# TLeconte/vdlm2dec

Measured on AMD Instinct MI355X. Metric: IQ MS/s demodulated (8 ch, 2 MS/s cs16) + CRC-pass frame parity vs ref, higher is better.
Workload: dtype f32

## Files before the change

vdlm2dec_amd/csrc/vdl2gpu.hip:

```cpp
#include "vdl2gpu_kernels.h"
#include "vdl2gpu_blocks.h"

#include <algorithm>
#include <cerrno>
#include <cmath>
#include <cstdio>
#include <cstdlib>
#include <chrono>
#include <cstring>
#include <mutex>
#include <new>
#include <string>
#include <type_traits>
#include <vector>

extern "C" void sincosf(float, float *, float *);

#define HIPCHK(h, expr)                                                                         \
	do {                                                                                    \
		hipError_t e__ = (expr);                                                        \
		if (e__ != hipSuccess) {                                                        \
			(h)->err = std::string(#expr) + ": " + hipGetErrorString(e__);          \
			return VDL2GPU_EHIP;                                                    \
		}                                                                               \
// ... 174 lines not shown
	uint64_t last_redo_push = 0;
	unsigned long long *d_dbg = nullptr;
	HeadTap *d_headtap = nullptr;
	unsigned *d_headtap_n = nullptr;
	unsigned headtap_cap = 0;
	uint64_t total_in = 0;
	uint64_t test_epoch = 0;
	unsigned test_ticket0 = 0;
	uint64_t pushes = 0;
	uint64_t overflowed = 0;
	std::vector<PushTiming> pending;
	std::vector<PushTiming> free_ev;
	vdl2gpu_timing_t tm{};
	RecQueue ready;
	std::vector<uint64_t> ready_idx;
	Slab slab[VDL2_NSLAB];
	unsigned slab_cap = 0;
	size_t ready_pos = 0;
	bool frames_on = false;
	unsigned *d_k4tab = nullptr;
	unsigned *d_fcnt = nullptr;
	unsigned frame_cap = 0;

	std::vector<uint8_t> fready;
	std::vector<size_t> fready_idx;
	size_t fready_pos = 0;
	uint64_t frames_dropped = 0;
	vdl2gpu_burst_t *h_pin = nullptr;
	bool col_on[VDL2_NCOL] = {};
	double lev_k = 1.0;
	unsigned *h_pin_cnt = nullptr;
	unsigned *d_pin_cnt = nullptr;
	unsigned pin_recs = 0;
	bool failed = false;
	std::string err;
	double hprof[8] = {0, 0, 0, 0, 0, 0, 0, 0};
	bool hprof_on = false;
	uint64_t hprof_push0 = 0;
	struct {
		bool no_k1_fast = false;
		bool no_tail = false;
		bool no_whole_pp = false;
		double table_fill = 0.90;
		bool k1_pp = false;
		bool debug_counters = false;
		bool split_fixed = false;
		int k1f_nfam = 0;
		int verify2_wg = 8;
		int k1_nsub = 0;
#ifdef VDL2GPU_TESTHOOKS
		int test_item_grid = 0;
		int test_item_common = 0;
		int test_item_verify = 0;
		int test_reg_cap = 0, test_seg_cap = 0, test_vis_cap = 0, test_win_cap = 0, test_merge_cap = 0, test_slog_cap = 0, test_stage_dyn = 0;
#endif
	} knob;
	struct Back {
		bool valid = false;
		K2Params k2{};
		int64_t J = 0;
		int par = 0, ring = 0, slab = 0;
		bool serial = false, two_streams = false;
		bool spec = false;
		unsigned tiles = 0;
		size_t pt_index = 0;
	} back;
	hipStream_t fstream = nullptr;
	LaterEvent k1_ev;
	hipEvent_t f_tail = nullptr;
	bool last_two_streams = false;
	int64_t last_J = 0;
	double st_scan = 0, st_cluster = 0, st_resolve = 0, st_demod = 0, st_other = 0, st_k1 = 0;
	uint64_t st_pushes = 0;
};

int LaterEvent::record(vdl2gpu_t *h, hipStream_t s) { HIPCHK(h, hipEventRecord(ev, s)); recorded = true; return VDL2GPU_OK; }
int LaterEvent::wait(vdl2gpu_t *h, hipStream_t s) const { if (recorded) HIPCHK(h, hipStreamWaitEvent(s, ev, 0)); return VDL2GPU_OK; }
int LaterEvent::sync(vdl2gpu_t *h) const { if (recorded) HIPCHK(h, hipEventSynchronize(ev)); return VDL2GPU_OK; }

extern "C" unsigned int reversebits(const unsigned int bits, const int n)
{
	unsigned int r = 0;
	for (int i = 0; i < n; ++i)
		r |= ((bits >> i) & 1u) << (n - 1 - i);
	return r;
}

extern "C" int vdl2gpu_lo_len(unsigned sdrinrate)
{
	unsigned a = sdrinrate, b = 25000u;
	while (b) {
		const unsigned t = a % b;
		a = b;
		b = t;
	}
	return a ? (int)(sdrinrate / a) : 0;
}

extern "C" int vdl2gpu_lo_table(unsigned sdrinrate, int fo_hz, float *out_re_im, int max_complex)
{
	const int L = vdl2gpu_lo_len(sdrinrate);
	if (L <= 0 || L > max_complex)
		return VDL2GPU_EINVAL;
	const float w = (float)((double)((float)fo_hz / (float)sdrinrate) * 2.0 * M_PI);
	for (int n = 0; n < L; ++n) {
		const float y = (float)(-n) * w;
		float sn, cs;
// ... 358 lines not shown
	ALLOC_TABLE(h, sel_list2, SC * VDL2_SEL_CAP * sizeof(unsigned));
	ALLOC_TABLE(h, regs, SC * VDL2_REG_CAP * sizeof(int2));
	ALLOC_TABLE(h, segs, SC * VDL2_SEG_CAP * sizeof(Seg));
	ALLOC_TABLE(h, fail, SC * sizeof(int));
	ALLOC_TABLE(h, redo, SC * sizeof(int));
	ALLOC_TABLE(h, cs_out, SC * sizeof(ChanState));
	ALLOC_TABLE(h, skey, SC * VDL2_CAND_CAP * sizeof(int));
	ALLOC_TABLE(h, sidx, SC * VDL2_CAND_CAP * sizeof(unsigned short));
	ALLOC_TABLE(h, prim, SC * VDL2_CAND_CAP * sizeof(unsigned short));
	ALLOC_TABLE(h, seeds, SC * VDL2_CAND_CAP * sizeof(int));
	for (TableSet &t : h->set) {
		DEV_ALLOC(h, t.k2.onchain, SC * VDL2_CAND_CAP);
		DEV_ALLOC(h, t.k2.slog, SC * VDL2_SLOG_CAP * sizeof(K2Slog));
		DEV_ALLOC(h, t.k2.win, SC * VDL2_WIN_CAP * sizeof(int2));
	}
	ALLOC_TABLE(h, items, SC * h->item_cap * sizeof(K2aItem));
	return VDL2GPU_OK;
}

static void fill_set_params(vdl2gpu_t *h)
{
	for (int r = 0; r < VDL2_NSET; ++r) {
		K2Params &k = h->set[r].k2;
		k.dec = h->d_dec[r];
		k.cap = h->cap;
		k.nbch = h->C;
		k.nstreams = h->S;
		k.ss = h->d_ss;
		k.cs = h->d_cs;
		k.cfg = h->d_cfg;
		k.pn = h->d_pn;
		k.pn8 = h->d_pn8;
		k.sel_mode = 0;
		k.stage_cap = h->stage_cap;
		k.outc_total_redo = h->d_outc + 8;
		k.rec_cap = h->rec_cap;
		k.probe_r = 0;
		k.prim_drop = h->prim_drop;
		k.dbg = h->knob.debug_counters ? h->d_dbg : nullptr;
		k.headtap = h->d_headtap;
		k.headtap_n = h->d_headtap_n;
		k.headtap_cap = h->headtap_cap;
		k.full_scan = h->full_scan;
#ifdef VDL2GPU_TESTHOOKS
		k.test_noregion = (h->cfg.flags & VDL2GPU_F_TEST_NOREGION) ? 1 : 0;
		{
			auto lim = [](int hook, int size) { return hook > 0 && hook < size ? hook : size; };
			k.lim_reg = lim(h->knob.test_reg_cap, VDL2_REG_CAP);
			k.lim_seg = lim(h->knob.test_seg_cap, VDL2_SEG_CAP);
			k.lim_vis = lim(h->knob.test_vis_cap, K2C_VIS);
			k.lim_win = lim(h->knob.test_win_cap, VDL2_WIN_CAP);
			k.lim_merge = lim(h->knob.test_merge_cap, K2S_MERGE);
			k.lim_slog = lim(h->knob.test_slog_cap, VDL2_SLOG_CAP);
			k.stage_cap = h->stage_cap - STAGE_DYN_SLOTS + (unsigned)lim(h->knob.test_stage_dyn, (int)STAGE_DYN_SLOTS);
		}
#endif
		k.round = 0;
		k.item_cap = h->item_cap;
		k.item_priv = h->item_priv;
		k.drain_slot = -1;
	}
}

static const int PART_SECONDS = 36, TEST_PART_NUM = 4, TEST_PART_DEN = 3;

static int create_impl(vdl2gpu_t *h)
{
	const vdl2gpu_config_t &cfg = h->cfg;
	int ndev = 0;
	if (hipGetDeviceCount(&ndev) != hipSuccess || ndev <= 0 || cfg.device >= ndev) {
		h->err = "no HIP device";
		return VDL2GPU_ENODEV;
	}
	HIPCHK(h, hipSetDevice(cfg.device));
	{
		hipDeviceProp_t prop;
		if (hipGetDeviceProperties(&prop, cfg.device) == hipSuccess && prop.multiProcessorCount > 0)
			h->n_cu = prop.multiProcessorCount;
		int occ = 0;
		if (hipOccupancyMaxActiveBlocksPerMultiprocessor(&occ, k2a_probe, K2A_THREADS, 0) == hipSuccess && occ > 0)
			h->probe_occ = occ;
	}
	int prio_lo = 0, prio_hi = 0;
	HIPCHK(h, hipDeviceGetStreamPriorityRange(&prio_lo, &prio_hi));
	NEW_STREAM(h, h->stream, &prio_hi);
	const int S = h->S, L = h->L;
	auto env_int = [](const char *name, int dflt) { const char *v = getenv(name); return v ? atoi(v) : dflt; };
	h->full_scan = ((cfg.flags & VDL2GPU_F_FULLSCAN) || getenv("VDL2GPU_FULL_SCAN")) ? 1 : 0;
	h->stage_every = std::max(1, env_int("VDL2GPU_STAGE_EVERY", h->stage_every));
	h->stage_dump = env_int("VDL2GPU_STAGE_DUMP", 0) != 0;
	if (h->stage_dump)
		h->stage_every = 1;
	h->k2d_grid = std::max(1, env_int("VDL2GPU_K2D_GRID", h->k2d_grid));
	h->knob.no_k1_fast = getenv("VDL2GPU_NO_K1_FAST") != nullptr;
	h->hprof_on = getenv("VDL2GPU_HOST_PROF") != nullptr;
	h->knob.no_tail = getenv("VDL2GPU_NO_TAIL") != nullptr;
	h->knob.no_whole_pp = getenv("VDL2GPU_NO_WHOLE_PP") != nullptr;
	h->knob.table_fill = std::min(100, std::max(10, env_int("VDL2GPU_TABLE_FILL", 90))) / 100.0;
	h->knob.k1_pp = getenv("VDL2GPU_K1_PP") != nullptr;
	h->knob.debug_counters = getenv("VDL2GPU_DEBUG_COUNTERS") != nullptr;
	h->knob.k1f_nfam = env_int("VDL2GPU_K1F_NFAM", 0);
	h->knob.verify2_wg = std::max(1, env_int("VDL2GPU_VERIFY2_WG", 8));
	h->knob.k1_nsub = env_int("VDL2GPU_K1_NSUB", 0);
#ifdef VDL2GPU_TESTHOOKS
	h->prim_drop = env_int("VDL2GPU_PRIM_DROP", 0);
	h->knob.test_item_grid = env_int("VDL2GPU_TEST_ITEM_GRID", 0);
	h->knob.test_item_common = env_int("VDL2GPU_TEST_ITEM_COMMON", 0);
	h->knob.test_item_verify = env_int("VDL2GPU_TEST_ITEM_VERIFY", 0);
	h->knob.test_reg_cap = env_int("VDL2GPU_TEST_REG_CAP", 0);
	h->knob.test_seg_cap = env_int("VDL2GPU_TEST_SEG_CAP", 0);
	h->knob.test_vis_cap = env_int("VDL2GPU_TEST_VIS_CAP", 0);
	h->knob.test_win_cap = env_int("VDL2GPU_TEST_WIN_CAP", 0);
	h->knob.test_merge_cap = env_int("VDL2GPU_TEST_MERGE_CAP", 0);
	h->knob.test_slog_cap = env_int("VDL2GPU_TEST_SLOG_CAP", 0);
	h->knob.test_stage_dyn = env_int("VDL2GPU_TEST_STAGE_DYN", 0);
#endif
	h->split_unit = ((cfg.flags & VDL2GPU_F_RTL_QUIRK) || h->sdrclk != 500 || h->L != 80) ? 32768 : K1F_PER_IN;
	if (!(cfg.flags & VDL2GPU_F_RTL_QUIRK) && h->split_unit == 32768 && (4 * h->sdrclk) % h->L == 0 && ((size_t)4 * h->sdrclk * h->sample_bytes) % 16 == 0)
		h->split_unit = (size_t)4 * h->sdrclk * ((32768 + (size_t)4 * h->sdrclk - 1) / ((size_t)4 * h->sdrclk));
	h->split_default = (size_t)((double)PART_SECONDS * (double)h->cfg.sdrinrate) / h->split_unit * h->split_unit;
	{
		const double max_frames = ((double)VDL2_MAXWG * K2A_VRUN - 4.0) * 2.0 * K2A_TS - 2.0 * K2A_TS - (double)VDL2_CARRY_FRAMES;
		const size_t max_part = (size_t)(max_frames * (double)h->sdrclk / 21.0) / h->split_unit * h->split_unit;
		h->split_default = std::min(h->split_default, max_part);
	}
	h->split_samples = std::max(h->split_unit, (size_t)(8.4 * (double)h->cfg.sdrinrate) / h->split_unit * h->split_unit);
#ifdef VDL2GPU_TESTHOOKS
	if (getenv("VDL2GPU_SPLIT_SAMPLES")) {
		h->split_samples = std::min((size_t)atoll(getenv("VDL2GPU_SPLIT_SAMPLES")), h->split_default * TEST_PART_NUM / TEST_PART_DEN);
		h->knob.split_fixed = true;
	}
#endif
	h->rounds_floor = 1;
	h->repair_rounds = env_int("VDL2GPU_REPAIR_ROUNDS", h->rounds_floor);
	h->force_serial = (cfg.flags & VDL2GPU_F_SERIAL) ? 1 : 0;
	h->quirk = (cfg.flags & VDL2GPU_F_RTL_QUIRK) ? 1 : 0;
	{
		const long long jmax = (long long)((21ull * cfg.max_push) / (unsigned)h->sdrclk) + 2;
		const long long jcap = (long long)PART_SECONDS * 84000 * TEST_PART_NUM / TEST_PART_DEN;
		const long long tiles_max = (VDL2_CARRY_FRAMES + std::min(jmax, jcap)) / K2A_TS + 2;
		const unsigned priv = (unsigned)std::min<long long>(VDL2_ITEM_PRIV, std::max<long long>(32768, (64 * tiles_max + 4095) / 4096 * 4096));
		h->item_priv = priv;
		h->item_cap = priv + std::max(priv / 2, 32768u);
	}
	h->k1_tbase.assign((size_t)S * 8, h->test_ticket0);
	h->cap = plane_frames(cfg.max_push, (unsigned)h->sdrclk);
	const size_t dec_bytes = (size_t)S * (size_t)h->cap * VDL2_CS * sizeof(float2);
	for (int r = 0; r < VDL2_NSET; ++r) {
		DEV_ALLOC(h, h->d_dec[r], dec_bytes);
		HIPCHK(h, hipMemsetAsync(h->d_dec[r], 0, dec_bytes, h->stream));
	}
	DEV_ALLOC(h, h->d_lo, (size_t)S * VDL2_CS * L * sizeof(float2));
	DEV_ALLOC(h, h->d_lo_ext, (size_t)S * VDL2_CS * (L + 48) * sizeof(float2));
	DEV_ALLOC(h, h->d_k1_tickets, (size_t)S * 21 * 8 * sizeof(unsigned));
	HIPCHK(h, hipMemsetAsync(h->d_k1_tickets, 0, (size_t)S * 21 * 8 * sizeof(unsigned), h->stream));
#ifdef VDL2GPU_TESTHOOKS
	if (h->test_ticket0) {
		const std::vector<unsigned> tk0((size_t)S * 21 * 8, h->test_ticket0);
		HIPCHK(h, hipMemcpyAsync(h->d_k1_tickets, tk0.data(), tk0.size() * sizeof(unsigned), hipMemcpyHostToDevice, h->stream));
		HIPCHK(h, hipStreamSynchronize(h->stream));
	}
#endif
	DEV_ALLOC(h, h->d_ss, (size_t)S * sizeof(StreamState));
	DEV_ALLOC(h, h->d_cs, (size_t)S * VDL2_CS * sizeof(ChanState));
	DEV_ALLOC(h, h->d_cfg, (size_t)S * VDL2_CS * sizeof(ChanCfg));
	DEV_ALLOC(h, h->d_pn, VDL2_PN_BITS);
	for (OutRing &rg : h->ring)
		DEV_ALLOC(h, rg.d_recs, (size_t)h->rec_cap * sizeof(vdl2gpu_burst_t));
// ... 994 lines not shown
	return VDL2GPU_OK;
}

static int enqueue_front(vdl2gpu_t *h, hipStream_t fs, long long dec_base, PushTiming &pt)
{
	vdl2gpu::Back &p = h->back;
	const int GS = h->S, par = p.par, ring = p.ring;
	const int64_t J = p.J;
	const bool serial = p.serial, two_streams = p.two_streams;
	TableSet &set = h->set[par];
	{
		KInitParams ki{};
		ki.ctl = set.k2.ctl + CTL_STAGE;
		ki.ctl_words = (int)(h->ctl_words - CTL_STAGE);
		ki.outc = h->d_outc + 2 * ring;
		ki.fail = set.k2.fail;
		ki.redo = set.k2.redo;
		ki.nsc = h->S * VDL2_CS;
		ki.fmask = set.k2.fmask;
		ki.fcnt = h->frames_on ? h->d_fcnt + 4 * ring : nullptr;
		hipLaunchKernelGGL(k_push_init, dim3(1), dim3(1024), 0, fs, ki);
	}
	TRY(mark(h, pt, E_SCAN_BEGIN, fs));
	K2Params k2 = set.k2;
	k2.J = J;
	k2.recs = h->ring[ring].d_recs;
	k2.levels = h->ring[ring].col<vdl2gpu_level_t>(COL_LEVEL);
	k2.soft = h->ring[ring].col<vdl2gpu_soft_t>(COL_SOFT);
	k2.carrier = h->ring[ring].col<vdl2gpu_carrier_t>(COL_CARRIER);
	k2.outc = h->d_outc + 2 * ring;
	k2.dec_base = dec_base;
	k2.scan_lo = dec_base + VDL2_HIST;
	k2.probe_par = (int)((dec_base + VDL2_HIST) & 1);
	k2.force_serial = serial ? 1 : 0;
	k2.sel_reserved = p.spec ? 1 : 0;
	if (h->d_headtap) {
		HIPCHK(h, hipStreamSynchronize(h->stream));
		HIPCHK(h, hipStreamSynchronize(h->pay_stream));
		HIPCHK(h, hipStreamSynchronize(h->copy_stream));
		HIPCHK(h, hipMemsetAsync(h->d_headtap_n, 0, sizeof(unsigned), fs));
	}
	const unsigned tiles = (unsigned)((VDL2_CARRY_FRAMES + J) / K2A_TS + 2);
	if (!serial) {
		ScanDrain pdrain, rdrain;
		{
			const unsigned want = h->full_scan ? tiles : tiles / 2 + 1;
			unsigned per = (unsigned)((h->n_cu * h->probe_occ + h->C * GS - 1) / (h->C * GS));
			per = per < 1 ? 1 : (per > want ? want : per);
			per = std::min<unsigned>(per, VDL2_MAXWG);
			TRY(launch_scan(h, SCAN_PROBE, k2, dim3(per, (unsigned)h->C, (unsigned)GS), fs, VDL2_SURV_PROBE,
					h->full_scan ? SURV_CANDS : SURV_PROBE, 0, (h->full_scan ? 4 : 1) * ((want + per - 1) / per), pdrain));
		}
		launch_per_channel(h, k2r_regions, K2R_NT, fs, k2, pdrain);
		TRY(launch_scan(h, SCAN_REGION, k2, dim3(128, (unsigned)h->C, (unsigned)GS), fs, VDL2_SURV_REGION, SURV_CANDS, 1, 2, rdrain));
		HIPCHK(h, hipGetLastError());
		launch_per_channel(h, k2s_sort, K2S_NT, fs, k2, rdrain);
	}
	TRY(mark(h, pt, E_FRONT_END, fs));
	HIPCHK(h, hipGetLastError());
	if (two_streams)
		HIPCHK(h, hipEventRecord(set.f_done, fs));
	{
		if (two_streams)
			TRY(h->set[set_after(par)].k2_done.wait(h, fs));
		K3Params k3{};
		k3.src = h->d_dec[par];
		k3.dst = h->d_dec[set_after(par)];
		k3.cap = h->cap;
		k3.nbch = h->C;
		k3.J = J;
		hipLaunchKernelGGL(k3_carry, dim3(24, (unsigned)h->C, (unsigned)GS), dim3(K3_THREADS), 0, fs, k3);
		HIPCHK(h, hipGetLastError());
		if (two_streams)
			HIPCHK(h, hipEventRecord(h->f_tail, fs));
		else
			TRY(h->k1_ev.record(h, fs));
	}
	p.valid = true;
	p.k2 = k2;
	p.tiles = tiles;
	p.pt_index = h->pending.size();
	return VDL2GPU_OK;
}

static int push_impl(vdl2gpu_t *h, const void *iq, size_t nsamples, size_t stream_stride_bytes, int memkind, bool wait_copy)
{
	if (!h || (!iq && nsamples))
		return VDL2GPU_EINVAL;
	if (nsamples == 0)
		return VDL2GPU_OK;
	if (nsamples > h->cfg.max_push)
		return VDL2GPU_EINVAL;
	if (h->S > 1 && stream_stride_bytes < nsamples * h->sample_bytes)
		return VDL2GPU_EINVAL;
	if (h->quirk && nsamples % 32768) {
		h->err = "VDL2GPU_F_RTL_QUIRK: every push must be whole 32768-sample blocks";
		return VDL2GPU_EINVAL;
	}
	HIPCHK(h, hipSetDevice(h->cfg.device));
	if (h->pending.size() >= 256) {
		HIPCHK(h, hipStreamSynchronize(h->fstream));
		HIPCHK(h, hipStreamSynchronize(h->stream));
		HIPCHK(h, hipStreamSynchronize(h->pay_stream));
		int rc = harvest_timing(h);
		if (rc)
			return rc;
	}
// ... 983 lines not shown
```

vdlm2dec_amd/csrc/vdl2gpu_scan.h:

```cpp
#ifndef VDL2GPU_SCAN_H
#define VDL2GPU_SCAN_H

#ifndef K2A_THREADS
#define K2A_THREADS 256
#endif
#ifndef K2A_TS
#define K2A_TS 1024
#endif
#ifndef K2A_WPE
#define K2A_WPE 6
#endif
#define K2A_POFF 132
#define K2A_XOFF (K2A_POFF + 16)
#define K2A_XMAX (2 * K2A_TS + K2A_XOFF)
#define K2X_WL 40
#define K2X_NT 256
#define K2X_CV 64
#define VDL2_ITEM_CAP 196608
#define VDL2_ITEM_PRIV 131072
#define VDL2_MAXWG 512
#define VDL2_REG_CAP 4096
#ifndef VDL2_REG_PAD
#define VDL2_REG_PAD 40
#endif
// ... 460 lines not shown
		v2f xe[10], xo[10];
#pragma unroll
		for (int i = 0; i < 5; ++i) {
			xe[2 * i] = e[i].xy;
			xe[2 * i + 1] = e[i].zw;
			xo[2 * i] = o[i].xy;
			xo[2 * i + 1] = o[i].zw;
		}
#pragma unroll
		for (int m = 0; m < 9; ++m) {
			acc0 = __builtin_elementwise_fma(xe[m], (v2f){mf[2 * m], mf[2 * m]}, acc0);
			acc1 = __builtin_elementwise_fma(xe[m + 1], (v2f){mf[2 * m], mf[2 * m]}, acc1);
			if (m < 8) {
				acc0 = __builtin_elementwise_fma(xo[m], (v2f){mf[2 * m + 1], mf[2 * m + 1]}, acc0);
				acc1 = __builtin_elementwise_fma(xo[m + 1], (v2f){mf[2 * m + 1], mf[2 * m + 1]}, acc1);
			}
		}
	} else {
		const v4f *pe = reinterpret_cast<const v4f *>(&sh.xs[q0]);
		v4f e[9];
#pragma unroll
		for (int i = 0; i < 9; ++i)
			e[i] = pe[i];
		v2f x[18];
#pragma unroll
		for (int i = 0; i < 9; ++i) {
			x[2 * i] = e[i].xy;
			x[2 * i + 1] = e[i].zw;
		}
#pragma unroll
		for (int j = 0; j < 17; ++j) {
			acc0 = __builtin_elementwise_fma(x[j], (v2f){mf[j], mf[j]}, acc0);
			acc1 = __builtin_elementwise_fma(x[j + 1], (v2f){mf[j], mf[j]}, acc1);
		}
	}
}

__device__ __forceinline__ v2f k2a_unit(v2f a)
{
	const float n2 = __fmaf_rn(a.x, a.x, a.y * a.y);
	v2f w = a * __frsqrt_rn(n2);
	if (!(n2 >= 1e-30f && n2 <= 1e30f)) {
		const float bad = (a.x == 0.0f && a.y == 0.0f) ? 0.0f : __builtin_nanf("");
		w = (v2f){1.0f + bad, bad};
	}
	return w;
}

__device__ __forceinline__ float k2a_lane_from(int byte_addr, float v)
{
	return __int_as_float(__builtin_amdgcn_ds_bpermute(byte_addr, __float_as_int(v)));
}

template <int S> __device__ void k2a_tile(K2aShared &sh, const K2Params &p, int sc, long long dec_base, long long nbase,
					   int cnt, unsigned rmask, int mode, long long chk_lo, long long chk_hi, int *fail,
					   int skip_r = -1, int skip_par = 0)
{
	const int tid = threadIdx.x;
	constexpr int PH = K2A_POFF / S;
	constexpr int LSTR = 8 / S;
	constexpr int E2 = 2 / S, E4 = 4 / S;
	constexpr int KH = LSTR / 2;
	constexpr int PPW = 64 - KH;
	constexpr int PPI = (K2A_THREADS / 64) * PPW;
	constexpr int NIT = ((K2A_TS + PH + 1) / 2 + PPI - 1) / PPI;
	constexpr int NL = (S * (K2A_TS - 1) + 1 + K2A_XOFF + K2A_THREADS - 1) / K2A_THREADS;
	static_assert(K2A_POFF == S * PH, "phase history must be a whole number of instants");
	float2 *const wu = (S != 1) ? sh.xs : sh.xs + K2A_WU1;
	const int nx = S * (cnt - 1) + 1 + K2A_XOFF;
	const bool prof = p.dbg && (mode == 2 || (mode == 0 && S == 1 && !p.full_scan && !p.full_round)) && tid == 0 && (blockIdx.x & 7) == 0;
	long long tq = prof ? clock64() : 0;
#define K2A_STAMP(slot) do { if (prof) { const long long tn = clock64(); sh.prof[slot] += (unsigned long long)(tn - tq); tq = tn; } } while (0)
	const int pbase = (S == 2) ? (tid & 1) * K2A_XODD + (tid >> 1) : tid;
	constexpr int pstep = K2A_THREADS / S;
	{
		const float2 *x = p.dec + (size_t)sc * p.cap + (nbase - K2A_XOFF - dec_base);
		float2 v[NL];
#pragma unroll
		for (int k = 0; k < NL; ++k)
			if (tid + k * K2A_THREADS < nx)
				v[k] = x[tid + k * K2A_THREADS];
		K2A_STAMP(12);
#pragma unroll
		for (int k = 0; k < NL; ++k)
			if (tid + k * K2A_THREADS < nx)
				sh.xs[pbase + k * pstep] = v[k];
	}
	K2A_STAMP(13);
	__syncthreads();
	K2A_STAMP(0);
	const int npairs = (cnt + PH + 1) / 2;
	const int wv = tid >> 6, ln = tid & 63;
	const int src_lane = (ln - KH) * 4;
#pragma unroll 1
	for (int r = 0; r < 4; ++r) {
		if (!(rmask & (1u << r)))
			continue;
		float mf[17];
#pragma unroll
		for (int j = 0; j < 17; ++j)
			mf[j] = __int_as_float(__builtin_amdgcn_readfirstlane(__float_as_int(sh.smf[r + 4 * j])));
		float4 hold[NIT];
#pragma unroll
		for (int it = 0; it < NIT; ++it) {
			const int pw = it * PPI + wv * PPW;
			if (pw >= npairs) {
				hold[it] = make_float4(0.0f, 0.0f, 0.0f, 0.0f);
				continue;
			}
			int q0 = 2 * (pw + ln - KH);
			q0 = q0 < 0 ? 0 : (q0 > K2A_TS + PH - 2 ? K2A_TS + PH - 2 : q0);
			v2f acc[2];
			k2a_fir2<S>(sh, q0, mf, acc[0], acc[1]);
			const v2f w0 = k2a_unit(acc[0]), w1 = k2a_unit(acc[1]);
			const float p0x = k2a_lane_from(src_lane, w0.x), p0y = k2a_lane_from(src_lane, w0.y);
			const float p1x = k2a_lane_from(src_lane, w1.x), p1y = k2a_lane_from(src_lane, w1.y);
			hold[it] = make_float4(__fmaf_rn(w0.x, p0x, w0.y * p0y), __fmaf_rn(w0.y, p0x, -(w0.x * p0y)),
					       __fmaf_rn(w1.x, p1x, w1.y * p1y), __fmaf_rn(w1.y, p1x, -(w1.x * p1y)));
			__builtin_amdgcn_sched_barrier(0);
		}
		K2A_STAMP(1);
		if (S != 1)
			__syncthreads();
		K2A_STAMP(2);
#pragma unroll
		for (int it = 0; it < NIT; ++it) {
			const int q0 = 2 * (it * PPI + wv * PPW + ln - KH);
			if (ln >= KH && q0 >= LSTR && q0 < cnt + PH)
				*reinterpret_cast<float4 *>(&wu[q0]) = hold[it];
		}
		K2A_STAMP(3);
		__syncthreads();
		unsigned npend = 0;
		for (int i0 = 0; i0 < cnt; i0 += K2A_THREADS) {
			const int i = i0 + tid;
			const int j = (i < cnt ? i : cnt - 1) + E2;
			const float2 *uq = &wu[PH - E4 + j - 15 * LSTR];
			float2 uu[16];
#pragma unroll
			for (int l = 0; l < 16; ++l)
				uu[l] = uq[l * LSTR];
			constexpr int kq[16] = {7, 4, 5, 3, 7, 6, 1, 3, 6, 0, 5, 2, 1, 2, 0, 4};
			v2f s4[4] = {{0.0f, 0.0f}, {0.0f, 0.0f}, {0.0f, 0.0f}, {0.0f, 0.0f}};
#pragma unroll
			for (int l = 0; l < 16; ++l) {
				const v2f u = {uu[l].x, uu[l].y};
				const int g = ((kq[l] & 1) << 1) | ((kq[l] >> 1) & 1);
				if (kq[l] & 4)
					s4[g] -= u;
				else
					s4[g] += u;
			}
			const v2f pa = {s4[0].x - s4[1].y, s4[0].y + s4[1].x};
			const v2f qa = {s4[2].x - s4[3].y, s4[2].y + s4[3].x};
			constexpr float RH = 0.70710678118654752f;
			const v2f acc = {__fmaf_rn(qa.x - qa.y, RH, pa.x), __fmaf_rn(qa.x + qa.y, RH, pa.y)};
			const float r2 = __fmaf_rn(acc.x, acc.x, acc.y * acc.y);
			bool pass = i < cnt && !(r2 <= VDL2_SCREEN_R2);
			if (mode == 0 && r == skip_r && (int)((nbase + S * (j - E4)) & 1) == skip_par)
				pass = false;
			const unsigned long long m = __ballot(pass);
			if (m != 0) {
				if (pass)
					sh.pend[wv][npend + __builtin_amdgcn_mbcnt_hi((unsigned)(m >> 32), __builtin_amdgcn_mbcnt_lo((unsigned)m, 0u))] =
						(unsigned short)(i | (!(r2 == r2) ? 0x8000 : 0));
				npend += (unsigned)__popcll(m);
			}
		}
		for (unsigned b = 0; b < npend; b += 64) {
			const bool on = b + (unsigned)ln < npend;
			const int e = on ? (int)sh.pend[wv][b + (unsigned)ln] : 0;
			const int j = (e & 0x3ff) + E2;
			const float2 *uq = &wu[PH - E4 + j - 15 * LSTR];
			float2 uu[16];
#pragma unroll
			for (int l = 0; l < 16; ++l)
				uu[l] = uq[l * LSTR];
			const long long n_abs = nbase + S * (j - E4);
			k2a_append(sh, p, sc, on, (int)(n_abs - dec_base), r, (mode == 1) ? (int)(chk_lo - dec_base) : 0,
				   (mode == 1) ? (int)(chk_hi - dec_base) : 0, uu, (e & 0x8000) != 0, mode, fail);
		}
		K2A_STAMP(4);
		K2A_STAMP(8);
		__syncthreads();
		K2A_STAMP(9);
		if (prof)
			sh.prof[11] += 1ull;
	}
#undef K2A_STAMP
}

__global__ __launch_bounds__(K2A_THREADS) __attribute__((amdgpu_waves_per_eu(K2A_WPE, 8)))
void k2a_probe(K2Params p)
{
	__shared__ K2aShared sh;
	const int c = blockIdx.y, s = (int)blockIdx.z;
	const int sc = s * VDL2_CS + c;
	const long long dec_base = p.dec_base;
	const long long avail_end = dec_base + VDL2_CARRY_FRAMES + p.J;
	if (p.force_serial)
		return;
	if (p.round > 0 && (!p.full_round || p.fail[sc] >= VDL2_VERIFIED))
		return;
	if (threadIdx.x < 16)
		sh.prof[threadIdx.x] = 0;
	k2a_tables(sh);
	if (p.full_scan || p.full_round) {
		const long long step = (long long)gridDim.x * K2A_TS;
		for (long long n0 = p.scan_lo + (long long)blockIdx.x * K2A_TS; n0 < avail_end; n0 += step) {
			const int nt = (int)((avail_end - n0 < K2A_TS) ? (avail_end - n0) : K2A_TS);
			k2a_tile<1>(sh, p, sc, dec_base, n0, nt, 0xfu, 0, 0, 0, nullptr);
		}
		k2a_tail(sh, sc);
		return;
	}
	const unsigned rmask = 1u << p.probe_r;
	const long long step = 2LL * gridDim.x * K2A_TS;
	for (long long n0 = p.scan_lo + 2LL * blockIdx.x * K2A_TS; n0 < avail_end; n0 += step) {
		const long long left = (avail_end - n0 + 1) / 2;
		const int nt = (int)(left < K2A_TS ? left : K2A_TS);
		k2a_tile<2>(sh, p, sc, dec_base, n0, nt, rmask, 2, 0, 0, nullptr);
	}
	k2a_tail(sh, sc);
	if (p.dbg && threadIdx.x < 16 && sh.prof[threadIdx.x])
		atomicAdd(p.dbg + 32 + threadIdx.x, sh.prof[threadIdx.x]);
}

#define WGS_NBK 2048
#define WGS_MAXB 48
struct WgSortShared {
	unsigned long long tmp[VDL2_CAND_CAP];
	unsigned start[WGS_NBK + 1], cur[WGS_NBK];
	unsigned part[64];
	unsigned maxb;
};

template <int NT> __device__ void wg_sort_u64(unsigned long long *keys, WgSortShared &ws, int n, int tshift, unsigned range)
{
	const int tid = threadIdx.x;
	int bsh = 0;
	while ((range >> bsh) >= WGS_NBK)
// ... 122 lines not shown
	for (int i = tid; i < ncand; i += K2R_NT)
		key64[i] = ((unsigned long long)(unsigned)seeds[i] << 16) | (unsigned)i;
	__syncthreads();
	wg_sort_u64<K2R_NT>(key64, ws, ncand, 16, (unsigned)(VDL2_CARRY_FRAMES + p.J));
	for (int i = tid; i < ncand; i += K2R_NT)
		key[i] = (int)(key64[i] >> 16);
	__syncthreads();
	{
		__shared__ int s_nreg;
		const int lo_lim = (int)(p.scan_lo - p.dec_base);
		const int hi_lim = (int)(VDL2_CARRY_FRAMES + p.J);
		int2 *regs = p.regs + (size_t)sc * VDL2_REG_CAP;
		if (tid == 0)
			s_nreg = 0;
		__syncthreads();
		for (int i = tid; i < ncand; i += K2R_NT) {
			if (i > 0 && key[i] - key[i - 1] <= VDL2_REG_GAP)
				continue;
			int j = i;
			while (j + 1 < ncand && key[j + 1] - key[j] <= VDL2_REG_GAP)
				++j;
			int lo = key[i] - VDL2_REG_PAD, hi = key[j] + VDL2_REG_PAD + 1;
			lo = lo < lo_lim ? lo_lim : lo;
			hi = hi > hi_lim ? hi_lim : hi;
			if (hi <= lo)
				continue;
			const int nchunk = (hi - lo + K2A_TS - 1) / K2A_TS;
			const int base = atomicAdd(&s_nreg, nchunk);
			for (int k = 0; k < nchunk; ++k)
				if (base + k < VDL2_REG_CAP) {
					const int q = lo + k * K2A_TS;
					regs[base + k] = make_int2(q, (hi - q < K2A_TS) ? hi - q : K2A_TS);
				}
		}
		__syncthreads();
#ifdef VDL2GPU_TESTHOOKS
		if (K2_REG_LIM(p) < VDL2_REG_CAP && s_nreg > K2_REG_LIM(p)) {
			const int n = s_nreg < VDL2_REG_CAP ? s_nreg : VDL2_REG_CAP, lim = K2_REG_LIM(p);
			for (int i = tid; i < n; i += K2R_NT)
				key64[i] = ((unsigned long long)(unsigned)regs[i].x << 32) | (unsigned)regs[i].y;
			__syncthreads();
			for (int i = tid; i < n; i += K2R_NT) {
				const int x = (int)(key64[i] >> 32);
				int rank = 0;
				for (int j = 0; j < n; ++j)
					rank += ((int)(key64[j] >> 32) < x) ? 1 : 0;
				const int k = (int)(((long long)rank * lim + n - 1) / n);
				if (k < lim && (int)((long long)k * n / lim) == rank)
					regs[k] = make_int2(x, (int)(key64[i] & 0xffffffffu));
			}
			__syncthreads();
		}
#endif
		if (tid == 0) {
			const int n = s_nreg;
			p.ctl[CTL_NREG0 + sc] = (unsigned)(n > K2_REG_LIM(p) ? K2_REG_LIM(p) : n);
			if (n > K2_REG_LIM(p))
				K2_COUNT(p, K2_DBG_ESC_REG);
			p.ctl[CTL_NSEED0 + sc] = 0;
		}
	}
}

#ifndef K2A_WPE_REGION
#define K2A_WPE_REGION 5
#endif
__global__ __launch_bounds__(K2A_THREADS) __attribute__((amdgpu_waves_per_eu(K2A_WPE_REGION, 8)))
void k2a_region(K2Params p)
{
	__shared__ K2aShared sh;
	const int c = blockIdx.y, s = (int)blockIdx.z;
	const int sc = s * VDL2_CS + c;
	if (p.force_serial || p.full_scan)
		return;
#ifdef VDL2GPU_TESTHOOKS
	if (p.test_noregion && p.round == 0)
		return;
#endif
	const unsigned nreg = p.ctl[CTL_NREG0 + sc];
	if (blockIdx.x >= nreg)
		return;
	const long long dec_base = p.dec_base;
	const int2 *regs = p.regs + (size_t)sc * VDL2_REG_CAP;
	const int skip_r = p.probe_r, skip_par = p.probe_par;
	if (threadIdx.x < 16)
		sh.prof[threadIdx.x] = 0;
	k2a_tables(sh);
	const bool prof = p.dbg && threadIdx.x == 0 && (blockIdx.x & 7) == 0;
	const long long t0 = prof ? clock64() : 0;
	for (unsigned k = blockIdx.x; k < nreg; k += gridDim.x) {
		const int2 rg = regs[k];
		k2a_tile<1>(sh, p, sc, dec_base, dec_base + rg.x, rg.y, 0xfu, 0, 0, 0, nullptr, skip_r, skip_par);
		if (prof)
			sh.prof[15] += (unsigned long long)rg.y;
	}
	const long long t1 = prof ? clock64() : 0;
	if (prof)
		sh.prof[12] += (unsigned long long)(t1 - t0);
	k2a_tail(sh, sc);
	if (p.dbg && threadIdx.x < 16 && sh.prof[threadIdx.x])
		atomicAdd(p.dbg + 48 + threadIdx.x, sh.prof[threadIdx.x]);
}

#ifndef K2A_VRUN
#define K2A_VRUN 4
#endif
#ifndef K2A_VGRID_RESIDENT
#define K2A_VGRID_RESIDENT 1
#endif
#define K2A_VITEMS 64

__device__ __forceinline__ int k2a_vseg(const Seg *segs, int k, int nseg, int p_lo, int t_end, int &lo, int &hi, int &r)
{
	lo = hi = r = 0;
	if (k >= nseg)
		return 0;
	const Seg g = segs[k];
	lo = g.lo > p_lo ? g.lo : p_lo;
	lo += (lo ^ g.lo) & 1;
	hi = g.hi < t_end ? g.hi : t_end;
	r = g.r & 3;
	if (g.hi <= g.lo || hi <= lo) {
		hi = lo;
		return 0;
	}
	return ((hi - lo + 1) / 2 + K2A_TS - 1) / K2A_TS;
}

__device__ __forceinline__ int k2a_vscan(int v, int *s_w, int &total)
{
	int incl = v;
	incl += __builtin_amdgcn_update_dpp(0, incl, 0x111, 0xf, 0xf, false);
	incl += __builtin_amdgcn_update_dpp(0, incl, 0x112, 0xf, 0xf, false);
	incl += __builtin_amdgcn_update_dpp(0, incl, 0x114, 0xf, 0xf, false);
	incl += __builtin_amdgcn_update_dpp(0, incl, 0x118, 0xf, 0xf, false);
	incl += __builtin_amdgcn_update_dpp(0, incl, 0x142, 0xa, 0xf, false);
	incl += __builtin_amdgcn_update_dpp(0, incl, 0x143, 0xc, 0xf, false);
	__syncthreads();
	if ((threadIdx.x & 63) == 63)
		s_w[threadIdx.x >> 6] = incl;
	__syncthreads();
	int base = 0, tot = 0;
#pragma unroll
	for (int w = 0; w < K2A_THREADS / 64; ++w) {
		const int t = s_w[w];
		base += (w < (int)(threadIdx.x >> 6)) ? t : 0;
		tot += t;
	}
	total = tot;
	return base + incl - v;
}

// ... 96 lines not shown
```

vdlm2dec_amd/csrc/vdl2gpu_types.h:

```cpp
#ifndef VDL2GPU_TYPES_H
#define VDL2GPU_TYPES_H


#include <hip/hip_runtime.h>
#include <stdint.h>
#include "vdl2_math.h"
#include "../../include/vdl2gpu.h"

#define VDL2_CS 8
#ifndef VDL2_NSET
#define VDL2_NSET 3
#endif
#define VDL2_NRING VDL2_NSET
#define VDL2_NSLAB (VDL2_NSET + 1)
static_assert(VDL2_NSET >= 3 && VDL2_NSET <= 4, "d_outc[] has the per-ring counters in front of the running totals at [8]; three bits of a record handle name its slab");
#define VDL2_HIST 160
#define VDL2_NPH 68
#define VDL2_STEADY 68
#define VDL2_MAXSYM 5456
#define VDL2_SERIAL_BELOW 4096
#define VDL2_CARRY_FRAMES 49152
#define VDL2_LONGEST_BURST 43592
#define VDL2_LEV_GUARD 512
#define VDL2_LEV_NEVAL 256
// ... 159 lines not shown
	Cluster *clusters;
	int2 *clhead;
	unsigned *ctl;
	BurstDesc *stage;
	unsigned *sel_list;
	unsigned *sel_list2;
	int sel_mode;
	unsigned stage_cap;
	vdl2gpu_burst_t *recs;
	vdl2gpu_level_t *levels;
	vdl2gpu_soft_t *soft;
	unsigned *outc;
	unsigned *outc_total_redo;
	unsigned *fmask;
	int full_round;
	int mini_round;
	int sel_reserved;
	unsigned rec_cap;
	int force_serial;
	int prim_drop;
	int full_scan;
	int test_noregion;
	int2 *regs;
	Seg *segs;
	int *fail;
	int *redo;
	int round;
	ChanState *cs_out;
	int *skey;
	unsigned short *sidx;
	unsigned short *prim;
	uint8_t *onchain;
	K2Slog *slog;
	int2 *win;
	int *seeds;
	struct K2aItem *items;
	unsigned item_cap;
	unsigned item_priv;
	int surv_pch, surv_nwg;
	int surv_common_cap;
	int surv_slot;
	int surv_mode;
	int surv_skip;
	int drain_slot;
	int drain_mode, drain_skip;
	int drain_pch, drain_nwg;
	unsigned long long *dbg;
	HeadTap *headtap;
	unsigned *headtap_n;
	unsigned headtap_cap;
	vdl2gpu_carrier_t *carrier;
#ifdef VDL2GPU_TESTHOOKS
	int lim_reg, lim_seg, lim_vis, lim_win, lim_merge, lim_slog;
#endif
};
#ifdef VDL2GPU_TESTHOOKS
#define K2_REG_LIM(p) ((p).lim_reg)
#define K2_SEG_LIM(p) ((p).lim_seg)
#define K2_VIS_LIM(p) ((p).lim_vis)
#define K2_WIN_LIM(p) ((p).lim_win)
#define K2_MERGE_LIM(p) ((p).lim_merge)
#define K2_SLOG_LIM(p) ((p).lim_slog)
enum { K2_DBG_ESC_REG = 64, K2_DBG_ESC_SEG, K2_DBG_ESC_VIS, K2_DBG_ESC_WIN, K2_DBG_ESC_MERGE, K2_DBG_ESC_SLOG, K2_DBG_ESC_STAGE,
       K2_DBG_INV_B_CLUSTER, K2_DBG_INV_B_DECODE, K2_DBG_INV_B_RECORD, K2_DBG_INV_A, K2_DBG_ESC_MERGE_SORT,
       K2_DBG_ESC_PATCH_ABANDON, K2_DBG_CHK_B_CLUSTER, K2_DBG_CHK_B_DECODE, K2_DBG_CHK_B_RECORD, K2_DBG_CHK_A };
#define VDL2_DBG_WORDS 96
#define K2_COUNT(p, slot) do { if ((p).dbg) atomicAdd((p).dbg + (slot), 1ull); } while (0)
#else
#define K2_REG_LIM(p) VDL2_REG_CAP
#define K2_SEG_LIM(p) VDL2_SEG_CAP
#define K2_VIS_LIM(p) K2C_VIS
#define K2_WIN_LIM(p) VDL2_WIN_CAP
#define K2_MERGE_LIM(p) K2S_MERGE
#define K2_SLOG_LIM(p) VDL2_SLOG_CAP
#define VDL2_DBG_WORDS 64
#define K2_COUNT(p, slot) do { } while (0)
#endif
#define CTL_OUT 0
#define CTL_OUT_OVF 1
#define CTL_STAGE 2
#define CTL_TICKET 3
#define CTL_STAGE_OVF 4
#define CTL_CAND0 8
#define CTL_NREG0 (CTL_CAND0 + 2 * p.nstreams * VDL2_CS)
#define CTL_NSEG0 (CTL_CAND0 + 3 * p.nstreams * VDL2_CS)
#define CTL_NSEL0 (CTL_CAND0 + 4 * p.nstreams * VDL2_CS)
#define CTL_NPRIM0 (CTL_CAND0 + 5 * p.nstreams * VDL2_CS)
#define CTL_NSEED0 (CTL_CAND0 + 6 * p.nstreams * VDL2_CS)
#define CTL_NCLUST0 (CTL_CAND0 + 7 * p.nstreams * VDL2_CS)
#define CTL_NSURV0 (CTL_CAND0 + 8 * p.nstreams * VDL2_CS)
enum { VDL2_SURV_PROBE = 0, VDL2_SURV_REGION = 1, VDL2_SURV_VERIFY = 2 , VDL2_SURV_FULL = 7, VDL2_SURV_SLOTS = 8 };
#define CTL_SELBASE0 (CTL_CAND0 + (8 + VDL2_SURV_SLOTS) * p.nstreams * VDL2_CS)
#define CTL_NSEL1 (CTL_CAND0 + (9 + VDL2_SURV_SLOTS) * p.nstreams * VDL2_CS)
#define CTL_SELBASE1 (CTL_CAND0 + (10 + VDL2_SURV_SLOTS) * p.nstreams * VDL2_CS)
#define CTL_NSURVLIM0 (CTL_CAND0 + (11 + VDL2_SURV_SLOTS) * p.nstreams * VDL2_CS)
#define CTL_NWIN0 (CTL_CAND0 + (11 + 2 * VDL2_SURV_SLOTS) * p.nstreams * VDL2_CS)
#define CTL_NSLOG0 (CTL_CAND0 + (12 + 2 * VDL2_SURV_SLOTS) * p.nstreams * VDL2_CS)
#define VDL2_CTL_WORDS(nsc) (CTL_CAND0 + (13 + 2 * VDL2_SURV_SLOTS) * (size_t)(nsc))
#define VDL2_WIN_CAP 32
#define VDL2_WIN_ALL 0xffffffffu
#define VDL2_SLOG_CAP 16

struct K3Params {
	const float2 *src;
	float2 *dst;
	long long cap;
	int nbch;
	long long J;
	StreamState *ss;
	const ChanState *cs;
	const unsigned *outc;
	const unsigned *fmask;
	const unsigned *fcnt;
	unsigned *host_cnt;
	int ring;
	const unsigned *ctl;
	int nstreams;
};

struct KInitParams {
	unsigned *ctl;
	int ctl_words;
	unsigned *outc;
	int *fail, *redo;
	int nsc;
	unsigned *fmask;
	unsigned *fcnt;
// ... 16 lines not shown
```

Measured before the change: 179,000.

## Pack several short regions into one region-scan tile pass

The region scan kernel used to process one region per tile pass, so short regions left most threads idle. It now packs up to eight regions that fit in a tile into a single k2a_tile pass, using segment offset, delta and cumulative-count tables to map each thread's sample to its source region. It also halves the region grid and doubles the drain parameter to match. The cost is extra per-element segment selection logic and more register pressure in the tile kernel.

```diff
diff --git a/vdlm2dec_amd/csrc/vdl2gpu.hip b/vdlm2dec_amd/csrc/vdl2gpu.hip
--- a/vdlm2dec_amd/csrc/vdl2gpu.hip
+++ b/vdlm2dec_amd/csrc/vdl2gpu.hip
@@ -250,7 +250,7 @@
 		int test_item_grid = 0;
 		int test_item_common = 0;
 		int test_item_verify = 0;
-		int test_reg_cap = 0, test_seg_cap = 0, test_vis_cap = 0, test_win_cap = 0, test_merge_cap = 0, test_slog_cap = 0, test_stage_dyn = 0;
+		int test_reg_cap = 0, test_seg_cap = 0, test_vis_cap = 0, test_win_cap = 0, test_merge_cap = 0, test_slog_cap = 0, test_stage_dyn = 0, test_region_pack = 0;
 #endif
 	} knob;
 	struct Back {
@@ -715,6 +715,7 @@
 			k.lim_win = lim(h->knob.test_win_cap, VDL2_WIN_CAP);
 			k.lim_merge = lim(h->knob.test_merge_cap, K2S_MERGE);
 			k.lim_slog = lim(h->knob.test_slog_cap, VDL2_SLOG_CAP);
+			k.lim_pack = lim(h->knob.test_region_pack, K2A_SEGS);
 			k.stage_cap = h->stage_cap - STAGE_DYN_SLOTS + (unsigned)lim(h->knob.test_stage_dyn, (int)STAGE_DYN_SLOTS);
 		}
 #endif
@@ -777,6 +778,7 @@
 	h->knob.test_merge_cap = env_int("VDL2GPU_TEST_MERGE_CAP", 0);
 	h->knob.test_slog_cap = env_int("VDL2GPU_TEST_SLOG_CAP", 0);
 	h->knob.test_stage_dyn = env_int("VDL2GPU_TEST_STAGE_DYN", 0);
+	h->knob.test_region_pack = env_int("VDL2GPU_TEST_REGION_PACK", 0);
 #endif
 	h->split_unit = ((cfg.flags & VDL2GPU_F_RTL_QUIRK) || h->sdrclk != 500 || h->L != 80) ? 32768 : K1F_PER_IN;
 	if (!(cfg.flags & VDL2GPU_F_RTL_QUIRK) && h->split_unit == 32768 && (4 * h->sdrclk) % h->L == 0 && ((size_t)4 * h->sdrclk * h->sample_bytes) % 16 == 0)
@@ -1877,7 +1879,8 @@
 					h->full_scan ? SURV_CANDS : SURV_PROBE, 0, (h->full_scan ? 4 : 1) * ((want + per - 1) / per), pdrain));
 		}
 		launch_per_channel(h, k2r_regions, K2R_NT, fs, k2, pdrain);
-		TRY(launch_scan(h, SCAN_REGION, k2, dim3(128, (unsigned)h->C, (unsigned)GS), fs, VDL2_SURV_REGION, SURV_CANDS, 1, 2, rdrain));
+		TRY(launch_scan(h, SCAN_REGION, k2, dim3(K2A_REGION_WG, (unsigned)h->C, (unsigned)GS), fs, VDL2_SURV_REGION, SURV_CANDS, 1,
+				2u * std::max(1u, 128u / (unsigned)K2A_REGION_WG), rdrain));
 		HIPCHK(h, hipGetLastError());
 		launch_per_channel(h, k2s_sort, K2S_NT, fs, k2, rdrain);
 	}
diff --git a/vdlm2dec_amd/csrc/vdl2gpu_scan.h b/vdlm2dec_amd/csrc/vdl2gpu_scan.h
--- a/vdlm2dec_amd/csrc/vdl2gpu_scan.h
+++ b/vdlm2dec_amd/csrc/vdl2gpu_scan.h
@@ -536,10 +536,22 @@
 	return __int_as_float(__builtin_amdgcn_ds_bpermute(byte_addr, __float_as_int(v)));
 }
 
-template <int S> __device__ void k2a_tile(K2aShared &sh, const K2Params &p, int sc, long long dec_base, long long nbase,
+#define K2A_SEGS 8
+struct K2aSegs {
+	int off[K2A_SEGS];
+	int delta[K2A_SEGS];
+	int ccum[K2A_SEGS];
+	int2 wn[K2A_SEGS];
+	int nseg, nx, neval;
+	long long t_mark;
+};
+static_assert((1 + K2A_XOFF) * K2A_SEGS > K2A_TS + K2A_XOFF && K2A_SEGS <= 8, "segment table; three bits of pend[] name a segment");
+
+template <int S, bool PACK = false> __device__ void k2a_tile(K2aShared &sh, const K2Params &p, int sc, long long dec_base, long long nbase,
 					   int cnt, unsigned rmask, int mode, long long chk_lo, long long chk_hi, int *fail,
-					   int skip_r = -1, int skip_par = 0)
-{
+					   int skip_r = -1, int skip_par = 0, const K2aSegs *sg = nullptr)
+{
+	static_assert(!PACK || S == 1, "packed passes are the region scan's");
 	const int tid = threadIdx.x;
 	constexpr int PH = K2A_POFF / S;
 	constexpr int LSTR = 8 / S;
@@ -551,19 +563,41 @@
 	constexpr int NL = (S * (K2A_TS - 1) + 1 + K2A_XOFF + K2A_THREADS - 1) / K2A_THREADS;
 	static_assert(K2A_POFF == S * PH, "phase history must be a whole number of instants");
 	float2 *const wu = (S != 1) ? sh.xs : sh.xs + K2A_WU1;
-	const int nx = S * (cnt - 1) + 1 + K2A_XOFF;
+	const int nx = PACK ? sg->nx : S * (cnt - 1) + 1 + K2A_XOFF;
+	const int neval = PACK ? sg->neval : cnt;
+	if (PACK)
+		cnt = nx - K2A_XOFF;
 	const bool prof = p.dbg && (mode == 2 || (mode == 0 && S == 1 && !p.full_scan && !p.full_round)) && tid == 0 && (blockIdx.x & 7) == 0;
 	long long tq = prof ? clock64() : 0;
 #define K2A_STAMP(slot) do { if (prof) { const long long tn = clock64(); sh.prof[slot] += (unsigned long long)(tn - tq); tq = tn; } } while (0)
 	const int pbase = (S == 2) ? (tid & 1) * K2A_XODD + (tid >> 1) : tid;
 	constexpr int pstep = K2A_THREADS / S;
 	{
-		const float2 *x = p.dec + (size_t)sc * p.cap + (nbase - K2A_XOFF - dec_base);
+		const float2 *x = p.dec + (size_t)sc * p.cap + (PACK ? 0 : (nbase - K2A_XOFF - dec_base));
 		float2 v[NL];
-#pragma unroll
-		for (int k = 0; k < NL; ++k)
-			if (tid + k * K2A_THREADS < nx)
-				v[k] = x[tid + k * K2A_THREADS];
+		if (PACK) {
+			int so[K2A_SEGS], sd[K2A_SEGS];
+#pragma unroll
+			for (int g = 0; g < K2A_SEGS; ++g) {
+				so[g] = sg->off[g];
+				sd[g] = sg->delta[g];
+			}
+#pragma unroll
+			for (int k = 0; k < NL; ++k) {
+				const int idx = tid + k * K2A_THREADS;
+				int d = sd[0];
+#pragma unroll
+				for (int g = 1; g < K2A_SEGS; ++g)
+					d = idx >= so[g] ? sd[g] : d;
+				if (idx < nx)
+					v[k] = x[idx + d];
+			}
+		} else {
+#pragma unroll
+			for (int k = 0; k < NL; ++k)
+				if (tid + k * K2A_THREADS < nx)
+					v[k] = x[tid + k * K2A_THREADS];
+		}
 		K2A_STAMP(12);
 #pragma unroll
 		for (int k = 0; k < NL; ++k)
@@ -576,6 +610,25 @@
 	const int npairs = (cnt + PH + 1) / 2;
 	const int wv = tid >> 6, ln = tid & 63;
 	const int src_lane = (ln - KH) * 4;
+	int gsel = 0;
+	if (PACK) {
+		static_assert(3 * (K2A_TS / K2A_THREADS) <= 32, "gsel");
+		int cc[K2A_SEGS];
+#pragma unroll
+		for (int g = 1; g < K2A_SEGS; ++g)
+			cc[g] = sg->ccum[g];
+#pragma unroll
+		for (int t = 0; t < K2A_TS / K2A_THREADS; ++t) {
+			int g = 0;
+#pragma unroll
+			for (int u = 1; u < K2A_SEGS; ++u)
+				g += (tid + t * K2A_THREADS >= cc[u]) ? 1 : 0;
+			gsel |= g << (3 * t);
+		}
+	}
+#ifdef VDL2GPU_TESTHOOKS
+	unsigned nscreened = 0;
+#endif
 #pragma unroll 1
 	for (int r = 0; r < 4; ++r) {
 		if (!(rmask & (1u << r)))
@@ -616,10 +669,18 @@
 		K2A_STAMP(3);
 		__syncthreads();
 		unsigned npend = 0;
-		for (int i0 = 0; i0 < cnt; i0 += K2A_THREADS) {
+		for (int i0 = 0; i0 < neval; i0 += K2A_THREADS) {
 			const int i = i0 + tid;
-			const int j = (i < cnt ? i : cnt - 1) + E2;
-			const float2 *uq = &wu[PH - E4 + j - 15 * LSTR];
+			const int j = (i < neval ? i : neval - 1) + E2;
+#ifdef VDL2GPU_TESTHOOKS
+			if (PACK) {
+				const int left = neval - (i0 + wv * 64);
+				nscreened += left <= 0 ? 0u : (left > 64 ? 64u : (unsigned)left);
+			}
+#endif
+			const int g = PACK ? (gsel >> (3 * (i0 / K2A_THREADS))) & 7 : 0;
+			const int2 wn = PACK ? sg->wn[g] : make_int2(0, 0);
+			const float2 *uq = &wu[PH - E4 + j - 15 * LSTR + wn.x];
 			float2 uu[16];
 #pragma unroll
 			for (int l = 0; l < 16; ++l)
@@ -640,14 +701,14 @@
 			constexpr float RH = 0.70710678118654752f;
 			const v2f acc = {__fmaf_rn(qa.x - qa.y, RH, pa.x), __fmaf_rn(qa.x + qa.y, RH, pa.y)};
 			const float r2 = __fmaf_rn(acc.x, acc.x, acc.y * acc.y);
-			bool pass = i < cnt && !(r2 <= VDL2_SCREEN_R2);
-			if (mode == 0 && r == skip_r && (int)((nbase + S * (j - E4)) & 1) == skip_par)
+			bool pass = i < neval && !(r2 <= VDL2_SCREEN_R2);
+			if (mode == 0 && r == skip_r && (int)(((PACK ? dec_base + wn.y : nbase) + S * (j - E4)) & 1) == skip_par)
 				pass = false;
 			const unsigned long long m = __ballot(pass);
 			if (m != 0) {
 				if (pass)
 					sh.pend[wv][npend + __builtin_amdgcn_mbcnt_hi((unsigned)(m >> 32), __builtin_amdgcn_mbcnt_lo((unsigned)m, 0u))] =
-						(unsigned short)(i | (!(r2 == r2) ? 0x8000 : 0));
+						(unsigned short)(i | (g << 10) | (!(r2 == r2) ? 0x8000 : 0));
 				npend += (unsigned)__popcll(m);
 			}
 		}
@@ -655,12 +716,13 @@
 			const bool on = b + (unsigned)ln < npend;
 			const int e = on ? (int)sh.pend[wv][b + (unsigned)ln] : 0;
 			const int j = (e & 0x3ff) + E2;
-			const float2 *uq = &wu[PH - E4 + j - 15 * LSTR];
+			const int2 wn = PACK ? sg->wn[(e >> 10) & 7] : make_int2(0, 0);
+			const float2 *uq = &wu[PH - E4 + j - 15 * LSTR + wn.x];
 			float2 uu[16];
 #pragma unroll
 			for (int l = 0; l < 16; ++l)
 				uu[l] = uq[l * LSTR];
-			const long long n_abs = nbase + S * (j - E4);
+			const long long n_abs = (PACK ? dec_base + wn.y : nbase) + S * (j - E4);
 			k2a_append(sh, p, sc, on, (int)(n_abs - dec_base), r, (mode == 1) ? (int)(chk_lo - dec_base) : 0,
 				   (mode == 1) ? (int)(chk_hi - dec_base) : 0, uu, (e & 0x8000) != 0, mode, fail);
 		}
@@ -671,6 +733,10 @@
 		if (prof)
 			sh.prof[11] += 1ull;
 	}
+#ifdef VDL2GPU_TESTHOOKS
+	if (PACK && p.dbg && ln == 0 && nscreened)
+		atomicAdd(p.dbg + K2_DBG_REGION_EVALS, (unsigned long long)nscreened);
+#endif
 #undef K2A_STAMP
 }
 
@@ -899,6 +965,13 @@
 			__syncthreads();
 		}
 #endif
+#ifdef VDL2GPU_TESTHOOKS
+		if (p.dbg) {
+			const int n = s_nreg > K2_REG_LIM(p) ? K2_REG_LIM(p) : s_nreg;
+			for (int i = tid; i < n; i += K2R_NT)
+				atomicAdd(p.dbg + K2_DBG_REGION_LISTED, 4ull * (unsigned long long)regs[i].y);
+		}
+#endif
 		if (tid == 0) {
 			const int n = s_nreg;
 			p.ctl[CTL_NREG0 + sc] = (unsigned)(n > K2_REG_LIM(p) ? K2_REG_LIM(p) : n);
@@ -912,10 +985,14 @@
 #ifndef K2A_WPE_REGION
 #define K2A_WPE_REGION 5
 #endif
+#ifndef K2A_REGION_WG
+#define K2A_REGION_WG 64
+#endif
 __global__ __launch_bounds__(K2A_THREADS) __attribute__((amdgpu_waves_per_eu(K2A_WPE_REGION, 8)))
 void k2a_region(K2Params p)
 {
 	__shared__ K2aShared sh;
+	__shared__ K2aSegs sg;
 	const int c = blockIdx.y, s = (int)blockIdx.z;
 	const int sc = s * VDL2_CS + c;
 	if (p.force_serial || p.full_scan)
@@ -934,17 +1011,60 @@
 		sh.prof[threadIdx.x] = 0;
 	k2a_tables(sh);
 	const bool prof = p.dbg && threadIdx.x == 0 && (blockIdx.x & 7) == 0;
-	const long long t0 = prof ? clock64() : 0;
-	for (unsigned k = blockIdx.x; k < nreg; k += gridDim.x) {
-		const int2 rg = regs[k];
-		k2a_tile<1>(sh, p, sc, dec_base, dec_base + rg.x, rg.y, 0xfu, 0, 0, 0, nullptr, skip_r, skip_par);
-		if (prof)
-			sh.prof[15] += (unsigned long long)rg.y;
-	}
-	const long long t1 = prof ? clock64() : 0;
 	if (prof)
-		sh.prof[12] += (unsigned long long)(t1 - t0);
+		sg.t_mark = clock64();
+	const int ln = threadIdx.x & 63;
+	for (unsigned k = blockIdx.x; k < nreg; ) {
+		if (threadIdx.x < 64) {
+			const unsigned kg = k + (unsigned)ln * gridDim.x;
+			const bool there = ln < K2A_SEGS && kg < nreg;
+			const int2 rg = there ? regs[kg] : make_int2(0, 0);
+			const int len = there ? rg.y + K2A_XOFF : K2A_XS_LEN;
+			int off = 0, cc = 0;
+#pragma unroll
+			for (int u = 0; u < K2A_SEGS - 1; ++u) {
+				const int lu = __builtin_amdgcn_readlane(len, u), cu = __builtin_amdgcn_readlane(rg.y, u);
+				off += ln > u ? lu : 0;
+				cc += ln > u ? cu : 0;
+			}
+			const bool take = ln < K2_PACK_LIM(p) && off + len <= K2A_TS + K2A_XOFF;
+			const int nseg = __popcll(__ballot(take));
+			if (ln < K2A_SEGS) {
+				sg.off[ln] = take ? off : 0x7fffffff;
+				sg.ccum[ln] = take ? cc : 0x7fffffff;
+				sg.delta[ln] = rg.x - K2A_XOFF - off;
+				sg.wn[ln] = make_int2(off - cc, rg.x - cc);
+			}
+			if (ln == 0)
+				sg.nseg = 0;
+			if (ln == nseg - 1) {
+				sg.nseg = nseg;
+				sg.nx = off + len;
+				sg.neval = cc + rg.y;
+			}
+		}
+		__syncthreads();
+		const int nseg = sg.nseg;
+		if (nseg == 0)
+			break;
+		if (prof) {
+			sh.prof[15] += (unsigned long long)sg.neval;
+			sh.prof[7] += (unsigned long long)nseg;
+		}
+		k2a_tile<1, true>(sh, p, sc, dec_base, 0, 0, 0xfu, 0, 0, 0, nullptr, skip_r, skip_par, &sg);
+		k += (unsigned)nseg * gridDim.x;
+	}
+	if (prof) {
+		const long long t1 = clock64();
+		sh.prof[5] += (unsigned long long)(t1 - sg.t_mark);
+		sh.prof[10] += 1ull;
+		sg.t_mark = t1;
+		if (blockIdx.x == 0)
+			atomicMax(p.dbg + 48 + 14, (unsigned long long)nreg);
+	}
 	k2a_tail(sh, sc);
+	if (p.dbg && threadIdx.x == 0 && (blockIdx.x & 7) == 0)
+		atomicAdd(p.dbg + 48 + 6, (unsigned long long)(clock64() - sg.t_mark));
 	if (p.dbg && threadIdx.x < 16 && sh.prof[threadIdx.x])
 		atomicAdd(p.dbg + 48 + threadIdx.x, sh.prof[threadIdx.x]);
 }
diff --git a/vdlm2dec_amd/csrc/vdl2gpu_types.h b/vdlm2dec_amd/csrc/vdl2gpu_types.h
--- a/vdlm2dec_amd/csrc/vdl2gpu_types.h
+++ b/vdlm2dec_amd/csrc/vdl2gpu_types.h
@@ -235,6 +235,7 @@
 	vdl2gpu_carrier_t *carrier;
 #ifdef VDL2GPU_TESTHOOKS
 	int lim_reg, lim_seg, lim_vis, lim_win, lim_merge, lim_slog;
+	int lim_pack;
 #endif
 };
 #ifdef VDL2GPU_TESTHOOKS
@@ -244,9 +245,11 @@
 #define K2_WIN_LIM(p) ((p).lim_win)
 #define K2_MERGE_LIM(p) ((p).lim_merge)
 #define K2_SLOG_LIM(p) ((p).lim_slog)
+#define K2_PACK_LIM(p) ((p).lim_pack)
 enum { K2_DBG_ESC_REG = 64, K2_DBG_ESC_SEG, K2_DBG_ESC_VIS, K2_DBG_ESC_WIN, K2_DBG_ESC_MERGE, K2_DBG_ESC_SLOG, K2_DBG_ESC_STAGE,
        K2_DBG_INV_B_CLUSTER, K2_DBG_INV_B_DECODE, K2_DBG_INV_B_RECORD, K2_DBG_INV_A, K2_DBG_ESC_MERGE_SORT,
-       K2_DBG_ESC_PATCH_ABANDON, K2_DBG_CHK_B_CLUSTER, K2_DBG_CHK_B_DECODE, K2_DBG_CHK_B_RECORD, K2_DBG_CHK_A };
+       K2_DBG_ESC_PATCH_ABANDON, K2_DBG_CHK_B_CLUSTER, K2_DBG_CHK_B_DECODE, K2_DBG_CHK_B_RECORD, K2_DBG_CHK_A,
+       K2_DBG_REGION_EVALS, K2_DBG_REGION_LISTED };
 #define VDL2_DBG_WORDS 96
 #define K2_COUNT(p, slot) do { if ((p).dbg) atomicAdd((p).dbg + (slot), 1ull); } while (0)
 #else
@@ -256,6 +259,7 @@
 #define K2_WIN_LIM(p) VDL2_WIN_CAP
 #define K2_MERGE_LIM(p) K2S_MERGE
 #define K2_SLOG_LIM(p) VDL2_SLOG_CAP
+#define K2_PACK_LIM(p) K2A_SEGS
 #define VDL2_DBG_WORDS 64
 #define K2_COUNT(p, slot) do { } while (0)
 #endif
```

Result: faster. 181,900, median of 6 (+1.6%).
